# EMI-Group/evogp

Measured on AMD Instinct MI355X. Metric: tree_evals_per_s, higher is better.
Workload: dtype f32; 1 GPU; BASELINE north_star / configs[2] shape: SymbolicRegression synthetic 10-var, GLOBAL pop=1000000 x 1024 datapoints, max_tree_len=64, funcs + - * /, one tree_SR_fitness pass over every rank's shard per step; global_pop=1000000, pop_per_gpu=1000000, datapoints=1024, var_len=10, max_tree_len=64, ranks=1, device_prewarm_calls=40

## Files before the change

evogp_amd/_lib.py:

```python
from __future__ import annotations

import ctypes as C
import os

_HERE = os.path.dirname(os.path.abspath(__file__))
LIB_PATH = os.environ.get("EVOGP_HIP_LIB") or os.path.join(_HERE, "lib", "libevogp_hip.so")

ABI_VERSION = 9

_vp = C.c_void_p
_u = C.c_uint
_i = C.c_int
_f = C.c_float

PROTOTYPES = {
    "evogp_hip_generate": [_u, _u, _u, _u, _u, _f, _f, _vp, _vp, _vp, _vp, _vp, _vp, _vp, _u, _vp],
    "evogp_hip_mutate": [_i, _i, _vp, _vp, _vp, _vp, _vp, _vp, _vp, _vp, _vp, _vp, _vp],
    "evogp_hip_crossover": [_i, _i, _i, _vp, _vp, _vp, _vp, _vp, _vp, _vp, _vp, _vp, _vp, _vp],
    "evogp_hip_evaluate": [_u, _u, _u, _u, _vp, _vp, _vp, _vp, _vp, _vp],
    "evogp_hip_sr_fitness": [_u, _u, _u, _u, _u, _i, _vp, _vp, _vp, _vp, _vp, _vp, _u, _vp],
    "evogp_hip_generate_masked": [_u, _u, _u, _u, _u, _f, _f, _vp, _vp, _vp, _vp, _vp, _vp, _vp, _u, _vp, _u, _vp],
    "evogp_hip_breed_default": [_i, _i, _i, _i, _vp, _vp, _vp, _vp, _vp, _u, _vp, _vp, _vp, _vp, _vp, _vp, _vp, _vp],
    "evogp_hip_breed_default_rows": [_i, _i, _i, _i, _vp, _vp, _vp, _vp, _vp, _u, _vp, _vp, _vp, _vp, _vp, _vp, _vp, _i, _i, _vp],
    "evogp_hip_breed_default_table": [_i, _i, _i, _i, _i, _vp, _vp, _vp, _vp, _vp, _u, _vp, _vp, _vp, _vp, _vp, _vp, _vp, _i, _i, _vp],
# ... 34 lines not shown
    "evogp_hip_tree_hash": [_u, _u, _vp, _vp, _vp, _vp, _vp],
    "evogp_hip_tree_classes_workspace_bytes": [_u, C.POINTER(C.c_ulonglong)],
    "evogp_hip_tree_classes": [_u, _u, _vp, _vp, _vp, _vp, _vp, _vp, _vp],
    "evogp_hip_sr_semantic_hash_workspace_bytes": [_u, C.POINTER(C.c_ulonglong)],
    "evogp_hip_sr_semantic_hash": [_u, _u, _u, _u, _u, _vp, _vp, _vp, _vp, _vp, _vp, _vp],
    "evogp_hip_sr_semantic_classes_workspace_bytes": [_u, C.POINTER(C.c_ulonglong)],
    "evogp_hip_sr_semantic_classes": [_u, _u, _u, _u, _u, _vp, _vp, _vp, _vp, _vp, _vp, _vp, _vp],
    "evogp_hip_sr_linear_scaling": [_u, _u, _u, _u, _u, _vp, _vp, _vp, _vp, _vp, _vp, _vp, _vp],
    "evogp_hip_sr_weighted_loss": [_u, _u, _u, _u, _u, _vp, _vp, _vp, _vp, _vp, _vp, _u, _i, C.c_double, _vp, _vp],
    "evogp_hip_sr_weighted_gradient": [_u, _u, _u, _u, _u, _vp, _vp, _vp, _vp, _vp, _vp, _i, C.c_double, _vp, _vp, _vp],
    "evogp_hip_sr_weighted_normal_eq": [_u, _u, _u, _u, _u, _vp, _vp, _vp, _vp, _vp, _vp, _vp, _vp, _vp],
    "evogp_hip_sr_weighted_scaling": [_u, _u, _u, _u, _u, _vp, _vp, _vp, _vp, _vp, _vp, _u, _vp, _vp, _vp],
    "evogp_hip_sr_input_gradient": [_u, _u, _u, _u, _u, _vp, _vp, _vp, _vp, _u, _vp, _vp, _vp, _vp],
    "evogp_hip_sr_derivative_loss": [_u, _u, _u, _u, _u, _vp, _vp, _vp, _vp, _vp, _vp, _u, _vp, _vp, _vp, _vp, _vp, _vp],
    "evogp_hip_sr_gene_fitness": [_u, _u, _u, _u, _u, _vp, _vp, _vp, _vp, _vp, _vp, _vp, _vp, _vp],
    "evogp_hip_wrap_linear":[_u, _u, _u, _vp, _vp, _vp, _vp, _vp, _vp, _vp, _vp, _vp],
    "evogp_hip_tree_intervals": [_u, _u, _u, _vp, _vp, _vp, _vp, _vp, _vp, _vp, _vp, _vp],
    "evogp_hip_tree_derivative_intervals": [_u, _u, _u, _vp, _vp, _vp, _vp, _vp, _u, _vp, _vp, _vp, _vp, _vp, _vp, _vp, _vp],
    "evogp_hip_tree_dimensions": [_u, _u, _u, _u, _vp, _vp, _vp, _vp, _vp, _i, _vp, _vp, _vp, _vp],
    "evogp_hip_tree_structure": [_u, _u, _u, _vp, _vp, _vp, _vp, _vp, _vp, _vp, _vp, _i, _i, _vp, _vp, _vp, _vp, _vp, _vp, _vp],
}

DEBUG_PROTOTYPES = {
    "evogp_hip_timer_begin": [_vp],
    "evogp_hip_timer_end": [_vp, C.POINTER(C.c_float)],
    "evogp_hip_debug_set_stats": [_vp],
    "evogp_hip_debug_compile_batch": [_i],
    "evogp_hip_debug_long_compiler": [_i],
    "evogp_hip_debug_twins": [_i],
    "evogp_hip_debug_tc_fold": [_i],
    "evogp_hip_debug_tc_end": [_i],
    "evogp_hip_debug_tc_nanpeek": [_i],
    "evogp_hip_debug_tc_nanpeek_raised": [],
    "evogp_hip_debug_tc_batches": [_i, _i],
    "evogp_hip_debug_tc_table": [_i],
    "evogp_hip_debug_tc_dense": [_i],
    "evogp_hip_debug_tc_dense_fallbacks": [],
    "evogp_hip_debug_tc_table_entry": [_i, _i, C.POINTER(C.c_uint)],
    "evogp_hip_debug_profile": [_i],
    "evogp_hip_debug_profile_read": [C.POINTER(C.c_float), C.POINTER(C.c_int)],
    "evogp_hip_debug_tc_histogram": [_u, _vp, _i, _vp],
    "evogp_hip_debug_tc_nhandlers": [],
    "evogp_hip_debug_tc_program": [_u, _vp, _i],
    "evogp_hip_debug_forget_function_classes": [],
    "evogp_hip_debug_structural_mutate_given": [_i, _i, _i, _i, _i, _vp, _vp, _vp, _vp, _vp, _vp, _vp, _vp],
    "evogp_hip_debug_insert_mutate_given": [_i, _i, _i, _vp, _vp, _vp, _vp, _vp, _vp, _vp, _vp, _vp, _vp, _vp],
    "evogp_hip_debug_point_mutate_given": [_i, _i, _i, _i, _i, _i, _i, _i, _i, _vp, _vp, _vp, _vp, _vp, _vp, _vp, _vp, _vp, _vp, _vp, _vp, _vp, _vp],
    "evogp_hip_debug_lexicase": [_vp, _i],
    "evogp_hip_debug_pareto_rank": [_i],
}


def _load() -> C.CDLL:
    if not os.path.exists(LIB_PATH):
        raise ImportError(
            f"{LIB_PATH} is missing: build the HIP engine first "
            "(python -c 'import __graft_entry__ as g; g.build()'  or  make -C evogp_amd/csrc). "
            "evogp_amd has no CPU fallback."
        )
    lib = C.CDLL(LIB_PATH)
    for name, argtypes in list(PROTOTYPES.items()) + list(DEBUG_PROTOTYPES.items()):
        fn = getattr(lib, name)
        fn.argtypes = argtypes
        fn.restype = _i
    lib.evogp_hip_evaluate_workspace_bytes.argtypes = [_u, _u]
    lib.evogp_hip_evaluate_workspace_bytes.restype = C.c_size_t
# ... 21 lines not shown
```

evogp_amd/csrc/gen/gen_tc_asm.py:

```python
#!/usr/bin/env python3
import os
import sys

sys.path.insert(0, os.path.dirname(os.path.abspath(__file__)))
from ocml_bodies import BODIES
from pair_rows import Pairing, check as check_pairing

FORMS = ("SS", "SV", "VS", "SC", "CS", "VV", "VC", "CV")
SENTINEL_HEAVY = 0x7FC0FEED
OPS = ("add", "sub", "mul", "div")
UNARY = ("neg", "abs", "sin", "cos", "tan", "sqrt", "lsqrt", "exp", "log", "llog")
GBIN = ("ldiv", "max", "min", "lt", "gt", "le", "ge", "pow", "lpow")
GUN = ("zero", "sinh", "cosh", "tanh", "one", "rcp")
HEAVY_REGS = 24
SLOT = 256
DIVIP_REGS = 12
DIVIP = ("SS", "SC", "CS")
DIVR = ("SV", "VV", "CV")
NOPF_TWINS = tuple(f"{op}_{form}" for op in ("add", "sub", "mul") for form in FORMS) + ("push_c", "push_v") \
    + tuple(f"divip_{f}" for f in DIVIP) + tuple(f"divr_{f}" for f in DIVR)
NHF = 37 + 2 * len(UNARY) + 8 + 2 + 4 + len(DIVIP) + 1 + 1 + len(DIVR) + len(NOPF_TWINS) + 1 + 3


NOPF = False
SPLAT = False
FMA_LOSS = False
PKARITH = True
DIVABREAST = True
PKCONST = True
TRUST = True
DIVFIX = False
DIVRANGE = True
DIV_LO, DIV_HI = 0x28800000, 0x56800000
EARLYREC = True
L2WARM = True
KWARM_LINES = 4
FUSED_SIZE_OFF, FUSED_LEN_OFF = 96 + 16, 96 + 60
TOUCH = True
TRIGPK = True
LIBPK = True
RECGLC = False
CODEWARM = False
CNDE64 = False
NANPEEK_BIT = 15
KWARM = False


def count_path(L, start, taken, idx_on=True, stop=()):
    idx = {line[:-1]: i for i, line in enumerate(L) if line.endswith(":")}
    c = {"valu": 0, "trans": 0, "salu": 0, "lds": 0, "vmem": 0, "smem": 0, "valu_clk": 0}
    i, steps = idx[start], 0
    while steps < 20000:
        steps += 1
        line = L[i]
        i += 1
        if line.endswith(":") and line[:-1] in stop:
            break
        if line.endswith(":") or line.startswith("."):
            continue
        w = line.split()
        op = w[0]
        if op.startswith("v_"):
            c["valu"] += 1
            if op.split("_")[1] in ("rcp", "sqrt", "exp", "log", "rsq", "sin", "cos"):
                c["trans"] += 1
                c["valu_clk"] += 8
            else:
                srcs = " ".join(w[2:]) if len(w) > 2 else ""
                fast = not idx_on and op in ("v_add_f32", "v_sub_f32", "v_subrev_f32", "v_mul_f32", "v_mov_b32") and not any(
                    t in srcs for t in ("s", "0x", "|", "%"))
                c["valu_clk"] += 2 if fast else 4
        elif op.startswith("ds_"):
            c["lds"] += 1
        elif op.startswith("global_") or op.startswith("buffer_"):
            c["vmem"] += 1
        elif op.startswith("s_load") or op.startswith("s_memtime"):
            c["smem"] += 1
# ... 112 lines not shown
            a(f"s_lshr_b32 {PF}, s{sX}, 24")

    def read_aux(dst):
        a(f"s_movrels_b32 s{dst}, s{W}")
        a(f"s_bfe_u32 s{dst}, s{dst}, 0x80010")

    def prefetch(nxt):
        if NOPF or twin[0]:
            return
        a(f"v_lshl_add_u32 v4, {PF}, 10, v2")
        read_bank(nxt, 4)

    def warm(sreg):
        if not L2WARM:
            return
        a(f"s_mul_hi_u32 s{T2}, {sreg}, s19")
        a(f"s_mul_i32 s{T1}, {sreg}, s19")
        a(f"s_add_u32 s{T1}, s{T1}, s8")
        a(f"s_addc_u32 s{T2}, s{T2}, s9")
        a(f"global_load_dwordx4 v[14:17], v13, s[{T1}:{T2}]")
        a(f"global_load_dwordx4 v[14:17], v13, s[{T1}:{T2}] offset:1024")

    LIVE = "%[karg]"

    def batch_size(end):
        a(f"s_sub_u32 s{sNB}, {end}, s{sT0}")
        dyn_batch(T1)
        a(f"s_min_u32 s{sNB}, s{sNB}, s{T1}")
        if peek:
            a(f"s_bfm_b64 {LIVE}, s{sNB}, 0")
            a(f"s_cmp_lt_u32 s{sNB}, 64")
            a(f"s_cselect_b64 {LIVE}, {LIVE}, -1")

    def peek_issue():
        skip = lab(f"no_peek_{len(sect[0])}")
        a(f"s_bitcmp1_b32 s17, {NANPEEK_BIT}")
        a(f"s_cbranch_scc0 {skip}")
        rec_addr(T1, T2, f"s{sT0}", T1)
        a("v_mul_lo_u32 v5, v0, s19")
        a(f"s_mov_b64 exec, {LIVE}")
        a(f"global_load_dword v18, v5, s[{T1}:{T2}]")
        a("s_mov_b64 exec, -1")
        a(f"{skip}:")

    def next_live(none):
        a(f"s_cmp_eq_u64 {LIVE}, 0")
        a(f"s_cbranch_scc1 {none}")
        a(f"s_ff1_i32_b64 s{sB}, {LIVE}")
        a(f"s_bitset0_b64 {LIVE}, s{sB}")

    def next_in_batch(none):
        if peek:
            a(f"s_cmp_eq_u64 {LIVE}, 0")
            a(f"s_cbranch_scc1 {none}")
            a(f"s_ff1_i32_b64 s{T2}, {LIVE}")
        else:
            a(f"s_add_u32 s{T2}, s{sB}, 1")
            a(f"s_cmp_lt_u32 s{T2}, s{sNB}")
            a(f"s_cbranch_scc0 {none}")

    def dyn_batch(dst):
        a(f"s_bfe_u32 s{T2}, s17, 0x20008")
        a(f"s_lshr_b32 s{dst}, s16, s{T2}")
        a(f"s_max_u32 s{dst}, s{dst}, 1")

    def grab():
        dyn_batch(T1)
        a("s_mov_b64 exec, 1")
        a(f"v_mov_b32 v9, s{T1}")
        a("global_atomic_add v12, v[10:11], v9, off sc0")
        a("s_mov_b64 exec, -1")

    def pool_grab():
        dyn_batch(T1)
# ... 66 lines not shown
        a(f"s_load_dwordx2 s[{P3_}:{P4_}], %[karg], 0x10")
        a("s_load_dwordx8 s[12:19], %[karg], 0x28")
        a("s_waitcnt lgkmcnt(0)")
        a(f"s_or_b32 s17, s17, {BASE}")
        a(f"v_mov_b32 v10, s{P3_}")
        a(f"v_mov_b32 v11, s{P4_}")
        a("s_mul_i32 s14, s14, s15")
        a(f"s_mul_i32 s14, s14, {G * 1024}")
        a("v_lshrrev_b32 v13, 4, v0")
        a("v_mul_lo_u32 v13, v13, s19")
        a("v_and_b32 v9, 15, v0")
        a("v_lshl_add_u32 v13, v9, 4, v13")
        a(f"s_load_dwordx4 s[{P1_}:{P4_}], %[karg], 0x48")
        a("s_waitcnt lgkmcnt(0)")
        a(f"s_mul_i32 {CUR}, {CUR}, s{P1_}")
        a(f"s_add_u32 {END_}, {CUR}, s{P1_}")
        a(f"s_mov_b32 {DYN}, s{P2_}")
        a(f"s_getreg_b32 s{P1_}, hwreg(HW_REG_XCC_ID, 0, 4)")
        a(f"s_bfe_u32 s{P2_}, s17, 0x3000c")
        a(f"s_and_b32 s{P1_}, s{P1_}, s{P2_}")
        a(f"s_mul_i32 s{P2_}, s{P1_}, s18")
        a(f"s_add_u32 {DYN}, {DYN}, s{P2_}")
        a(f"s_add_u32 s{P2_}, {DYN}, s18")
        a(f"s_min_u32 s12, s12, s{P2_}")
        a(f"s_lshl_b32 s{P1_}, s{P1_}, 7")
        a(f"v_add_co_u32 v10, vcc, s{P1_}, v10")
        a("v_addc_co_u32 v11, vcc, 0, v11, vcc")
        a(f"s_getpc_b64 s[{T1}:{T2}]")
        a(f"{lab('pc')}:")
        a(f"s_add_u32 s{T1}, s{T1}, {lab('hbase')}-{lab('pc')}")
        a(f"s_addc_u32 s{T2}, s{T2}, 0")
        a(f"s_mov_b32 {BASE}, s{T1}")
        a(f"s_mov_b32 s{sPC + 1}, s{T2}")
        if CODEWARM:
            a("v_lshlrev_b32 v4, 6, v0")
            a(f"s_mov_b32 s{P3_}, ({lab('code_end')}-{lab('hbase')}+4095)/4096")
            a(f"{lab('codewarm')}:")
            a(f"global_load_dword v14, v4, s[{T1}:{T2}]")
            a(f"s_add_u32 s{T1}, s{T1}, 4096")
            a(f"s_addc_u32 s{T2}, s{T2}, 0")
            a(f"s_sub_u32 s{P3_}, s{P3_}, 1")
            a(f"s_cmp_lg_u32 s{P3_}, 0")
            a(f"s_cbranch_scc1 {lab('codewarm')}")
        a(f"{lab('run')}:")
        if stats:
            for r in (A_REC, A_WORK, A_TREES, A_DISP):
                a(f"v_mov_b32 v{r}, 0")
            a(f"s_memtime s[{T1}:{T2}]")
            a("s_waitcnt lgkmcnt(0)")
            a(f"v_mov_b32 v{A_START}, s{T1}")
        a("s_mov_b32 s18, 1")
        pool_grab()
        a("s_waitcnt lgkmcnt(0)")
        a(f"v_readfirstlane_b32 s{sT0N}, v12")
        a(f"s_add_u32 s{sT0N}, s{sT0N}, {CUR}")
        a(f"{lab('batch')}:")
        a("s_cmp_eq_u32 s18, 0")
        a(f"s_cbranch_scc1 {lab('dyn')}")
        a(f"s_mov_b32 s{sT0}, s{sT0N}")
        a(f"s_cmp_lt_u32 s{sT0}, {END_}")
        a(f"s_cbranch_scc0 {lab('to_dyn')}")
        if peek:
            batch_size(END_)
            peek_issue()
        pool_grab()
        warm(f"s{sT0}")
# ... 4 lines not shown
        a("s_mov_b32 s18, 0")
        tick_begin()
        grab()
        a("s_waitcnt vmcnt(0)")
        tick_end(A_WORK)
        a(f"v_readfirstlane_b32 s{sT0N}, v12")
        a(f"s_add_u32 s{sT0N}, s{sT0N}, {DYN}")
        a(f"{lab('dyn')}:")
        a(f"s_mov_b32 s{sT0}, s{sT0N}")
        a(f"s_cmp_ge_u32 s{sT0}, s12")
        a(f"s_cbranch_scc1 {lab('exit')}")
        if peek:
            batch_size("s12")
            peek_issue()
        grab()
        warm(f"s{sT0}")
        if not peek:
            batch_size("s12")
    a(f"{lab('have_batch')}:")
    a(f"s_mov_b64 s[{sOK}:{sOK + 1}], 0")
    a("v_mov_b32 v7, 0")
    if peek:
        nw = 2 if L2WARM else 0
        a(f"s_mov_b32 s{sNB}, 0")
        a(f"s_bitcmp1_b32 s17, {NANPEEK_BIT}")
        a(f"s_cbranch_scc0 {lab('first_tree')}")
        a("s_cmp_eq_u32 s18, 1")
        a(f"s_cbranch_scc1 {lab('peek_pool')}")
        a(f"s_waitcnt vmcnt({nw + 1})")
        a(f"s_branch {lab('peek_here')}")
        a(f"{lab('peek_pool')}:")
        a(f"s_waitcnt vmcnt({nw})")
        a(f"{lab('peek_here')}:")
        a("v_and_b32 v18, 0xffff, v18")
        a(f"v_cmp_eq_u32 vcc, {hex(SLOT * hid['nan_tree'])}, v18")
        a("v_mov_b32 v9, 0x7fc00000")
        a(f"s_and_b64 vcc, vcc, {LIVE}")
        a(f"s_andn2_b64 {LIVE}, {LIVE}, vcc")
        a(f"s_mov_b64 s[{sOK}:{sOK + 1}], vcc")
        a("s_nop 1")
        a("v_cndmask_b32 v7, v7, v9, vcc")
        a(f"{lab('first_tree')}:")
        next_live(lab('batch_end'))
    else:
        a(f"s_mov_b32 s{sB}, 0")
    a(f"{lab('tree')}:")
    if fused:
        rec_addr(sREC, sREC + 1, f"s{sB}", T1)
    else:
        a(f"s_add_u32 s{T1}, s{sT0}, s{sB}")
        rec_addr(sREC, sREC + 1, f"s{T1}", T1)
    tick_begin()
    load_window()
    a(f"{lab('tree_loaded')}:")
    a("v_mov_b32 v6, 0")
    a(f"s_mov_b32 s{sTILE}, 0")
    a("s_waitcnt lgkmcnt(0)")
    tick_end(A_REC)
    if not fused:
        if peek:
            a(f"s_add_u32 s{sNB}, s{sNB}, 1")
            a(f"s_cmp_eq_u32 s{sNB}, 2")
        else:
            a(f"s_cmp_eq_u32 s{sB}, 1")
        a(f"s_cbranch_scc0 {lab('no_prewarm')}")
        a("s_cmp_eq_u32 s18, 1")
        a(f"s_cbranch_scc0 {lab('no_prewarm')}")
        second_tree_hook("", lab('no_prewarm'))
        a(f"{lab('no_prewarm')}:")
    if stats:
        a(f"v_add_u32 v{A_TREES}, 1, v{A_TREES}")
    elif KWARM and not fused:
        for i in range(KWARM_LINES):
            a(f"s_load_dwordx2 %[karg], s[{sREC}:{sREC + 1}], {hex(256 + 64 * i)}")
# ... 1625 lines not shown
        if x is not None:
            rows_op("sub", y, y, x)
        elif PKCONST and K >= 2:
            for k in range(0, K, 2):
                a(f"v_pk_add_f32 v[{y + k}:{y + k + 1}], v[{y + k}:{y + k + 1}], s[{sA}:{sA + 1}] op_sel_hi:[1,0] neg_lo:[0,1] neg_hi:[0,1]")
        else:
            for k in range(K):
                a(f"v_subrev_f32 v{y + k}, s{sA}, v{y + k}")
        rows_op("mul", y, y, y)
        for k in range(K):
            a(f"v_add_f32 v6, v6, v{y + k}")

    for fl in (0, 1):
        a(f"{lab(f'lean_last{fl}')}:")
        early_record(f"lean{fl}")
        rows_op("sub", S0, P[fl], S0)
        rows_op("mul", S0, S0, S0)
        for k in range(K):
            a(f"v_add_f32 v6, v6, v{S0 + k}")
        a(f"s_branch {lab('tree_done')}")
        a(f"{lab(f'lean_moved{fl}')}:")
        a("s_bitset0_b32 s17, 31")
        if fused:
            rec_addr(sREC, sREC + 1, f"s{sB}", T1)
        else:
            a(f"s_add_u32 s{T1}, s{sT0}, s{sB}")
            rec_addr(sREC, sREC + 1, f"s{T1}", T1)
        load_window()
        rows_op("mul", S0, S0, S0)
        for k in range(K):
            a(f"v_add_f32 v6, v6, v{S0 + k}")
        a("s_waitcnt lgkmcnt(0)")
        a(f"s_branch {lab('tile')}")
    for leaf in ("leaf_c", "leaf_v"):
        var = leaf == "leaf_v"
        Xb, Yb = ((P[0], P[1]) if var else (None, None)), (T, Q)
        for ph in (0, 1):
            a(f"{lab(f'{leaf}_p{ph}')}:")
            a(f"s_add_u32 s{sTILE}, s{sTILE}, 1")
            a(f"s_cmp_lt_u32 s{sTILE}, s15")
            a(f"s_cbranch_scc0 {lab(f'{leaf}_last{ph}')}")
            if var:
                a(f"v_add_u32 v4, {G * 1024}, v4")
                read_bank(Xb[1 - ph], 4)
            a(f"v_add_u32 v3, {G * 1024}, v3")
            read_bank(Yb[1 - ph], 3)
            a(f"s_waitcnt lgkmcnt({(2 if var else 1) * G})")
            mse_rows(Yb[ph], Xb[ph])
            if ph == 1:
                a(f"s_branch {lab(f'{leaf}_p0')}")
        for ph in (0, 1):
            a(f"{lab(f'{leaf}_last{ph}')}:")
            a("s_waitcnt lgkmcnt(0)")
            early_record(f"{leaf}{ph}")
            mse_rows(Yb[ph], Xb[ph])
            a(f"s_branch {lab('tree_done')}")

    for fl in (0, 1):
        Y = P[fl]
        a(f"{lab(f'endbody{fl}')}:")
        a("s_set_gpr_idx_off")
        if stats:
            pass
        a(f"s_add_u32 s{T1}, s{sTILE}, 1")
        a("s_waitcnt lgkmcnt(0)")
        if EARLYREC and not stats:
            a(f"s_cmp_lt_u32 s{T1}, s15")
            a(f"s_cbranch_scc1 {lab(f'no_early{fl}')}")
            next_in_batch(lab(f'no_early{fl}'))
            if not fused:
                a(f"s_add_u32 s{T2}, s{T2}, s{sT0}")
            rec_addr(sREC, sREC + 1, f"s{T2}", T2)
            load_window()
            a(f"{lab(f'no_early{fl}')}:")
        a(f"s_and_b32 s{T2}, s17, 0x12")
        a(f"s_cbranch_scc0 {lab(f'end_full{fl}')}")
        a(f"s_cmp_lt_u32 s{T1}, s15")
        a(f"s_cselect_b32 s{T2}, 0, s17")
        a("s_bitcmp1_b32 s17, 4")
        a(f"s_cselect_b32 s{T2}, s17, s{T2}")
        a(f"s_and_b32 s{T2}, s{T2}, 2")
        a("s_waitcnt lgkmcnt(0)")
        a(f"s_cmp_eq_u32 s{T2}, 0")
        a(f"s_cbranch_scc1 {lab(f'end_full{fl}')}")
        a(f"s_mul_i32 s{T2}, s{sTILE}, {64 * K}")
        a(f"v_mul_u32_u24 v5, {RPL}, v0")
        for k in range(K):
            g, q = divmod(k, 4)
            a(f"s_add_u32 s{T4}, s{T2}, {g * 256 + q}")
# ... 18 lines not shown
        else:
            for k in range(K):
                a(f"v_sub_f32 v{S0 + k}, v{Y + k}, v{S0 + k}")
            for k in range(K):
                a(f"v_mul_f32 v{S0 + k}, v{S0 + k}, v{S0 + k}")
            for k in range(K):
                a(f"v_add_f32 v6, v6, v{S0 + k}")
        a(f"s_branch {lab('end_acc')}")
        a(f"{lab(f'end_abs{fl}')}:")
        for k in range(K):
            a(f"v_sub_f32 v{S0 + k}, v{Y + k}, v{S0 + k}")
        for k in range(K):
            a(f"v_add_f32_e64 v6, v6, |v{S0 + k}|")
        if fl == 0:
            a(f"s_branch {lab('end_acc')}")
    a(f"{lab('end_acc')}:")
    a(f"s_mov_b32 s{sTILE}, s{T1}")
    a(f"s_cmp_lt_u32 s{sTILE}, s15")
    a(f"s_cbranch_scc0 {lab('tree_done')}")
    if fused:
        rec_addr(T1, T2, f"s{sB}", T1)
    else:
        a(f"s_add_u32 s{T1}, s{sT0}, s{sB}")
        rec_addr(T1, T2, f"s{T1}", T1)
    a(f"s_cmp_eq_u32 s{T1}, s{sREC}")
    a(f"s_cbranch_scc1 {lab('tile')}")
    a(f"s_mov_b32 s{sREC}, s{T1}")
    a(f"s_mov_b32 s{sREC + 1}, s{T2}")
    load_window()
    a("s_waitcnt lgkmcnt(0)")
    a(f"s_branch {lab('tile')}")
    a(f"{lab('tree_done')}:")
    a("s_bitset0_b32 s17, 31")
    for ctl in ("row_shr:1 row_mask:0xf bank_mask:0xf bound_ctrl:0", "row_shr:2 row_mask:0xf bank_mask:0xf bound_ctrl:0",
                "row_shr:4 row_mask:0xf bank_mask:0xf bound_ctrl:0", "row_shr:8 row_mask:0xf bank_mask:0xf bound_ctrl:0",
                "row_bcast:15 row_mask:0xa bank_mask:0xf", "row_bcast:31 row_mask:0xc bank_mask:0xf"):
        a("s_nop 1")
        a(f"v_add_f32_dpp v6, v6, v6 {ctl}")
    a("s_nop 1")
    a(f"v_readlane_b32 s{T1}, v6, 63")
    a(f"s_and_b32 s{T2}, s{T1}, 0x7fffffff")
    a(f"s_cmp_gt_u32 s{T2}, 0x7f800000")
    a(f"s_cselect_b32 s{T1}, 0x7fc00000, s{T1}")
    a(f"s_mov_b32 m0, s{sB}")
    a(f"s_bitset1_b64 s[{sOK}:{sOK + 1}], s{sB}")
    a(f"v_writelane_b32 v7, s{T1}, m0")
    if EARLYREC and not stats:
        if peek:
            next_live(lab('batch_end'))
        else:
            a(f"s_add_u32 s{sB}, s{sB}, 1")
            a(f"s_cmp_lt_u32 s{sB}, s{sNB}")
            a(f"s_cbranch_scc0 {lab('batch_end')}")
        a("s_bitcmp1_b32 s17, 10")
        a(f"s_cbranch_scc1 {lab('tree_loaded')}")
        a(f"s_branch {lab('tree')}")
    a(f"{lab('next_tree')}:")
    if peek:
        next_live(lab('batch_end'))
        a(f"s_branch {lab('tree')}")
    else:
        a(f"s_add_u32 s{sB}, s{sB}, 1")
        a(f"s_cmp_lt_u32 s{sB}, s{sNB}")
        a(f"s_cbranch_scc1 {lab('tree')}")
    a(f"{lab('batch_end')}:")
    if peek:
        a(f"s_bitcmp1_b32 s17, {NANPEEK_BIT}")
        a(f"s_cbranch_scc0 {lab('hooked')}")
        a(f"s_cmp_ge_u32 s{sNB}, 2")
        a(f"s_cbranch_scc1 {lab('hooked')}")
        a("s_cmp_eq_u32 s18, 1")
        a(f"s_cbranch_scc0 {lab('hooked')}")
        a("s_waitcnt lgkmcnt(0)")
        second_tree_hook("_end", lab('hooked'))
        a(f"{lab('hooked')}:")
    tick_begin()
    if fused:
        a("s_waitcnt vmcnt(0)")
    else:
# ... 176 lines not shown
```

evogp_amd/csrc/sr_tc.hip:

```cpp
#include "interp.hpp"
#include "launch.hpp"
#include "sr_params.hpp"
#include "tc_interp_k8.inc"
#include "tc_interp_k4.inc"
#include "tc_interp_k1.inc"

#include <atomic>
#include <cstddef>
#include <mutex>
#include <cstdio>
#include <vector>

namespace evogp {

struct TcCompileParams {
    const float *value;
    const int16_t *type;
    const int16_t *size;
    uint2 *prog;
    float *fitness;
    unsigned *marks;
    unsigned *zero_next;
    int pop, gp_len, var_len;
    uint32_t unary_mask;
// ... 6 lines not shown
    int nblocks;
    int rows;
    int general;
    int heavy_reserve;
    int div_reserve;
    int classify;
    uint32_t recip;
    int twins;
    int long_fast;
    int learn;
    int nan_trees;
    int end_id;
    int leaf_id;
};

__device__ inline uint32_t division_in_place(uint32_t id, int after, const TcCompileParams &p) {
    if (id < 24u || id >= 32u) return id;
    const uint32_t form = id - 24u;
    const uint32_t ip = form == 0u ? (uint32_t)EVOGP_TC_H_DIVIP_SS : form == 3u ? (uint32_t)EVOGP_TC_H_DIVIP_SC : form == 4u ? (uint32_t)EVOGP_TC_H_DIVIP_CS : 0u;
    if (ip == 0u) return id;
    const int before = after + (form == 0u ? 1 : 0);
    return before + p.div_reserve <= p.depth ? ip : id;
}

enum : int { TC_S = 0, TC_V = 1, TC_C = 2 };
constexpr int kMarkSampleBlocks = 64;
constexpr int kZeroRounds = 3;
static std::atomic<int> g_long_fast{-1};
static std::atomic<int> g_twins{-1};
static std::atomic<int> g_fold{-1};
static std::atomic<int> g_lean_end{-1};
static std::atomic<int> g_nanpeek{-1};
static std::atomic<int> g_nanpeek_raised{0};
static std::atomic<int> g_tc_batch{0}, g_tc_dynshift{-1};
static std::atomic<int> g_compile_batch{-2};
static std::atomic<int> g_word_table{-1};
static int tc_nan_trees() {
    static const int env_fold = env_int("EVOGP_TC_FOLD", 2);
    const int fo = g_fold.load(std::memory_order_relaxed);
    return fo >= 0 ? fo : (env_fold < 0 || env_fold > 2 ? 2 : env_fold);
}
static bool tc_lean_end() {
    static const int env_end = env_int("EVOGP_TC_END", 1);
    const int le = g_lean_end.load(std::memory_order_relaxed);
    return (le >= 0 ? le : env_end) != 0;
}
static bool tc_nanpeek(long n, int num_cus) {
    static const int env_peek = env_int("EVOGP_TC_NANPEEK", 1);
    const int np = g_nanpeek.load(std::memory_order_relaxed);
    return np >= 0 ? np != 0 : (env_peek == 2 || (env_peek == 1 && n >= 900l * num_cus));
}
static bool tc_word_table() {
    static const int env_table = env_int("EVOGP_TC_TABLE", 1);
    const int wt = g_word_table.load(std::memory_order_relaxed);
    return (wt >= 0 ? wt : env_table) != 0;
}
static std::atomic<int> g_dense{-1};
static bool tc_dense() {
    static const int env_dense = env_int("EVOGP_TC_DENSE", 1);
    const int de = g_dense.load(std::memory_order_relaxed);
    return (de >= 0 ? de : env_dense) != 0;
}
static std::atomic<unsigned *> g_dense_fallbacks{nullptr};
static_assert(EVOGP_TC_H_LEAF_V == EVOGP_TC_H_LEAF_C + 1, "TcCompileParams::leaf_id: the variable's word is the constant's + 1, as PUSH_V is PUSH_C + 1");
static_assert(kSentinelHeavy == 0x7FC0FEEDu, "gen/gen_tc_asm.py SENTINEL_HEAVY");

__device__ inline float fold_bin4_fast(int op, float x, float y) {
    return op == 0 ? x + y : op == 1 ? x - y : op == 2 ? x * y : (y == 0.0f ? __builtin_nanf("") : x / y);
}

__device__ inline uint32_t tc_word0(int id, int slot, uint32_t pf_bytes, uint32_t aux = 0u) {
    return ((pf_bytes >> 10) << 24) | ((aux & 0xFFu) << 16) | (uint32_t)(((slot & 1) * EVOGP_TC_NHANDLERS + id) * EVOGP_TC_SLOT);
}

static_assert(EVOGP_TC_H_PUSH_V == EVOGP_TC_H_PUSH_C + 1 && EVOGP_TC_H_DIVIP_CS == EVOGP_TC_H_DIVIP_SS + 2 && EVOGP_TC_H_DIVR_CV == EVOGP_TC_H_DIVR_SV + 2 &&
              EVOGP_TC_H_PUSH_C_NP == EVOGP_TC_H_ADD_SS_NP + 24 && EVOGP_TC_H_DIVIP_SS_NP == EVOGP_TC_H_ADD_SS_NP + 26 &&
              EVOGP_TC_H_DIVR_SV_NP == EVOGP_TC_H_ADD_SS_NP + 29, "gen/gen_tc_asm.py NOPF_TWINS");
__device__ inline int no_prefetch_delta(bool arith3, bool push_c, bool in_place, bool by_recip) {
    return arith3 ? (int)EVOGP_TC_H_ADD_SS_NP : push_c ? (int)EVOGP_TC_H_PUSH_C_NP - (int)EVOGP_TC_H_PUSH_C
         : in_place ? (int)EVOGP_TC_H_DIVIP_SS_NP - (int)EVOGP_TC_H_DIVIP_SS : by_recip ? (int)EVOGP_TC_H_DIVR_SV_NP - (int)EVOGP_TC_H_DIVR_SV : 0;
}
__device__ inline bool next_word_has_variable(const TcCompileParams &, unsigned long long keptwave, bool kept, bool uses_var, bool is_root) {
    const unsigned long long U = __ballot(kept & uses_var);
// ... 3247 lines not shown
        if (marks) {
            marks += (size_t)piece * kCallScratchChunkWords;
            t.counter = marks + 32;
            t.flags |= 1 << 16;
            regions = xcc_regions(stream);
            if (regions > kCallScratchXcds) regions = kCallScratchXcds;
            if ((env_xcc == 1 || env_xcc == 2 || env_xcc == 4 || env_xcc == 8) && env_xcc <= regions) regions = env_xcc;
        } else {
            t.counter = acquire_counter(strm, &le);
            if (!t.counter) return le;
        }
        long blocks = (long)info.num_cus * wgs_per_cu;
        const long grain = std::max(1, batch >> dyn_shift);
        const long need_blocks = ((long)n + grain * wg_waves - 1) / (grain * wg_waves);
        if (blocks > need_blocks) blocks = need_blocks;
        int static_pct = K == 1 ? 50 : n < 200000 ? 85 : 75;
        if (env_static >= 0 && env_static <= 100) static_pct = env_static;
        t.static_per_wg = (uint32_t)(((long)n * static_pct / 100) / blocks);
        t.dyn_start = t.static_per_wg * (uint32_t)blocks;
        t.waves_per_wg = (uint32_t)wg_waves;
        {
            const long tail = (long)n - (long)t.dyn_start;
            while (regions > 1 && (long)regions > blocks) regions >>= 1;
            if (tail < (long)regions * batch * 4) regions = 1;
            long per = (tail + regions - 1) / regions;
            per = (per + batch - 1) / batch * batch;
            t.reserved = (int)per;
            static_assert(kCallScratchXcds <= 8, "TcParams::flags bits 12-14");
            t.flags |= (regions - 1) << 12;
        }
        const bool may_divide = p.func_mask == 0u || (p.func_mask & (1u << F_DIV)) != 0u;
        if (!STATS && !WIDE && nan_words && may_divide && tc_nanpeek(n, info.num_cus)) t.flags |= 1 << 15;
        g_nanpeek_raised.store((t.flags >> 15) & 1, std::memory_order_relaxed);
        unsigned *publish = marks && piece == 0 && pieces == 1 && chunks == 1 && learn_packed ? p.feedback : nullptr;
        hipLaunchKernelGGL((sr_tc_kernel<K, STATS, FAST, WIDE>), dim3((unsigned)blocks), dim3(wg_waves * 64), lds, strm, t, publish, p.feedback_expected,
                           div_magic((unsigned)t.var_len), div_magic((t.pad & 0xFFFFu) > 0u ? (t.pad & 0xFFFFu) : 1u));
        return hipGetLastError();
    };

    if (p.classify) {
        int *cls = (int *)(records + cls_off);
        hipLaunchKernelGGL(tc_label_groups_kernel, dim3(1), dim3(1024), 0, stream, (const int *)p.y, p.D, p.out_len, K, piece_rows, (int)cls_q,
                           cls, cls + p.D, cls + p.D + cls_q);
        const int nxp = (int)cls_q * p.var_len;
        hipLaunchKernelGGL(tc_permute_rows_kernel, dim3((unsigned)((nxp + 1023) / 1024)), dim3(256), 0, stream, p.X, (const int *)(cls + p.D),
                           (float *)(cls + p.D + 2 * cls_q), p.var_len, nxp);
        if ((e = hipGetLastError()) != hipSuccess) return e;
    }
    if (chunks == 1) {
        if ((e = launch_compilers(0, p.pop, p.marks, true, stream)) != hipSuccess) return e;
        if (p.zero_next) call_scratch_next_is_clean(stream);
        if (p.prof_mid) (void)hipEventRecord(p.prof_mid, stream);
        for (int piece = 0; piece < pieces; ++piece)
            if ((e = launch_interpreter(0, p.pop, p.marks, stream, piece)) != hipSuccess) return e;
        if (pieces > 1 && !p.classify) {
            hipLaunchKernelGGL(tc_scale_kernel, dim3((unsigned)((p.pop + 255) / 256)), dim3(256), 0, stream, p.fitness, p.pop, (float)p.D);
            if ((e = hipGetLastError()) != hipSuccess) return e;
        }
    } else {
        if ((e = hipEventRecord(d.fork, stream)) != hipSuccess) return e;
        if ((e = hipStreamWaitEvent(d.side, d.fork, 0)) != hipSuccess) return e;
        for (int c = 0; c < chunks; ++c) {
            const int lo = (int)((long)p.pop * c / chunks), hi = (int)((long)p.pop * (c + 1) / chunks);
            unsigned *cm = p.marks + (size_t)c * kCallScratchChunkWords;
            if ((e = launch_compilers(lo, hi - lo, cm, c == 0, d.side)) != hipSuccess) return e;
            if ((e = hipEventRecord(d.ready[c], d.side)) != hipSuccess) return e;
// ... 330 lines not shown
extern "C" int evogp_hip_debug_twins(int mode) {
    if (mode < -1 || mode > 1) return EVOGP_E_BADARG;
    evogp::g_twins.store(mode, std::memory_order_relaxed);
    return EVOGP_OK;
}

extern "C" int evogp_hip_debug_tc_fold(int mode) {
    if (mode < -1 || mode > 2) return EVOGP_E_BADARG;
    evogp::g_fold.store(mode, std::memory_order_relaxed);
    return EVOGP_OK;
}

extern "C" int evogp_hip_debug_tc_end(int mode) {
    if (mode < -1 || mode > 1) return EVOGP_E_BADARG;
    evogp::g_lean_end.store(mode, std::memory_order_relaxed);
    return EVOGP_OK;
}

extern "C" int evogp_hip_debug_tc_nanpeek(int mode) {
    if (mode < -1 || mode > 1) return EVOGP_E_BADARG;
    evogp::g_nanpeek.store(mode, std::memory_order_relaxed);
    return EVOGP_OK;
}

extern "C" int evogp_hip_debug_tc_batches(int batch, int dyn_shift) {
    if (batch < 0 || batch > 64 || dyn_shift < -1 || dyn_shift > 3) return EVOGP_E_BADARG;
    evogp::g_tc_batch.store(batch, std::memory_order_relaxed);
    evogp::g_tc_dynshift.store(dyn_shift, std::memory_order_relaxed);
    return EVOGP_OK;
}

extern "C" int evogp_hip_debug_tc_nanpeek_raised(void) { return evogp::g_nanpeek_raised.load(std::memory_order_relaxed); }

extern "C" int evogp_hip_debug_tc_table(int mode) {
    if (mode < -1 || mode > 1) return EVOGP_E_BADARG;
    evogp::g_word_table.store(mode, std::memory_order_relaxed);
    return EVOGP_OK;
}

extern "C" int evogp_hip_debug_tc_dense(int mode) {
    if (mode < -1 || mode > 1) return EVOGP_E_BADARG;
    evogp::g_dense.store(mode, std::memory_order_relaxed);
    return EVOGP_OK;
}

extern "C" int evogp_hip_debug_tc_dense_fallbacks(void) {
    const unsigned *const word = evogp::g_dense_fallbacks.load(std::memory_order_relaxed);
    unsigned n = 0u;
    if (!word || hipDeviceSynchronize() != hipSuccess || hipMemcpy(&n, word, sizeof n, hipMemcpyDeviceToHost) != hipSuccess) return -1;
    return (int)n;
}

extern "C" int evogp_hip_debug_tc_table_entry(int recip, int code, unsigned *entry) {
    if (recip < 0 || recip > 1 || code < 0 || code >= evogp::kTcCodes || !entry) return EVOGP_E_BADARG;
    entry[0] = evogp::kTcWordTableHost.ids[recip][code];
    entry[1] = evogp::kTcWordTableHost.bits[recip][code];
    return EVOGP_OK;
}

extern "C" int evogp_hip_debug_long_compiler(int fast) {
    if (fast < -1 || fast > 1) return EVOGP_E_BADARG;
    evogp::g_long_fast.store(fast, std::memory_order_relaxed);
    return EVOGP_OK;
}

extern "C" int evogp_hip_debug_compile_batch(int trees) {
// ... 104 lines not shown
```

include/evogp_hip_debug.h:

```cpp
#ifndef EVOGP_HIP_DEBUG_H
#define EVOGP_HIP_DEBUG_H
#include "evogp_hip.h"
#ifdef __cplusplus
extern "C" {
#endif

int evogp_hip_timer_begin(evogp_stream_t stream);
int evogp_hip_timer_end(evogp_stream_t stream, float *elapsed_ms);

int evogp_hip_debug_set_stats(unsigned long long *device_counters);

int evogp_hip_debug_profile(int enable);
int evogp_hip_debug_profile_read(float *stage_ms , int *calls);

int evogp_hip_debug_compile_batch(int trees);
int evogp_hip_debug_long_compiler(int fast);
int evogp_hip_debug_twins(int mode);
int evogp_hip_debug_tc_fold(int mode);
int evogp_hip_debug_tc_end(int mode);
int evogp_hip_debug_tc_nanpeek(int mode);
int evogp_hip_debug_tc_nanpeek_raised(void);
int evogp_hip_debug_tc_batches(int batch, int dyn_shift);
int evogp_hip_debug_tc_table(int mode);
int evogp_hip_debug_tc_dense(int mode);
int evogp_hip_debug_tc_dense_fallbacks(void);
int evogp_hip_debug_tc_table_entry(int recip, int code, unsigned *entry);

int evogp_hip_debug_tc_histogram(unsigned pop, unsigned long long *device_hist, int hist_len, evogp_stream_t stream);
int evogp_hip_debug_tc_nhandlers(void);
int evogp_hip_debug_tc_program(unsigned tree, unsigned *host_words, int max_words);

int evogp_hip_debug_forget_function_classes(void);

int evogp_hip_debug_structural_mutate_given(int pop_size, int gp_len, int mode, int inner_is_offset, int skip_rows, const int *given,
                                            const float *value, const int16_t *type, const int16_t *size, float *value_res,
                                            int16_t *type_res, int16_t *size_res, evogp_stream_t stream);
int evogp_hip_debug_insert_mutate_given(int pop_size, int gp_len, int skip_rows, const int *given, const float *value, const int16_t *type,
                                        const int16_t *size, const float *donor_value, const int16_t *donor_type, const int16_t *donor_size,
                                        float *value_res, int16_t *type_res, int16_t *size_res, evogp_stream_t stream);
int evogp_hip_debug_point_mutate_given(int pop_size, int gp_len, int mode, int modify_output, int fix_roulette, int skip_rows, int input_len,
                                       int output_len, int n_consts, const unsigned char *target, const float *u, const int *var_idx,
                                       const int *const_idx, const int *out_idx, const float *value, const int16_t *type, const int16_t *size,
                                       const float *roulette_ufuncs, const float *roulette_bfuncs, const float *roulette_tfuncs,
                                       const float *const_samples, float *value_res, evogp_stream_t stream);

int evogp_hip_debug_lexicase(unsigned long long *device_counters, int stop_after);

int evogp_hip_debug_pareto_rank(int stop_after);

#ifdef __cplusplus
}
#endif
#endif
```

Baseline: 1990 billion tree-evals/s.

## Peek tree roots to batch-evaluate single-leaf trees in a dedicated walk loop

Extends the NaN-peek preload in the generated SR fitness assembly so it also spots trees whose root is a lone constant or variable leaf. It loads an extra word per tree and flags these trees, then evaluates them in a separate leaf-walk loop that reuses the leaf MSE tile bodies and skips the normal interpreter dispatch. The path is gated on population size and lean-end mode, and it can be toggled by an environment variable or a debug call. It adds code size and branch complexity, and it packs a flag into the low bit of the code base register.

```diff
diff --git a/evogp_amd/_lib.py b/evogp_amd/_lib.py
--- a/evogp_amd/_lib.py
+++ b/evogp_amd/_lib.py
@@ -90,6 +90,8 @@
     "evogp_hip_debug_tc_end": [_i],
     "evogp_hip_debug_tc_nanpeek": [_i],
     "evogp_hip_debug_tc_nanpeek_raised": [],
+    "evogp_hip_debug_tc_leafpeek": [_i],
+    "evogp_hip_debug_tc_leafpeek_raised": [],
     "evogp_hip_debug_tc_batches": [_i, _i],
     "evogp_hip_debug_tc_table": [_i],
     "evogp_hip_debug_tc_dense": [_i],
diff --git a/evogp_amd/csrc/gen/gen_tc_asm.py b/evogp_amd/csrc/gen/gen_tc_asm.py
--- a/evogp_amd/csrc/gen/gen_tc_asm.py
+++ b/evogp_amd/csrc/gen/gen_tc_asm.py
@@ -43,6 +43,7 @@
 CODEWARM = False
 CNDE64 = False
 NANPEEK_BIT = 15
+LEAFPEEK_PAD_BIT = 17
 KWARM = False
 
 
@@ -221,14 +222,23 @@
             a(f"s_cmp_lt_u32 s{sNB}, 64")
             a(f"s_cselect_b64 {LIVE}, {LIVE}, -1")
 
+    def leafpeek_test():
+        a(f"s_bitcmp1_b32 {BASE}, 0")
+
     def peek_issue():
-        skip = lab(f"no_peek_{len(sect[0])}")
+        skip, wide = lab(f"no_peek_{len(sect[0])}"), lab(f"peek_x2_{len(sect[0])}")
         a(f"s_bitcmp1_b32 s17, {NANPEEK_BIT}")
         a(f"s_cbranch_scc0 {skip}")
         rec_addr(T1, T2, f"s{sT0}", T1)
         a("v_mul_lo_u32 v5, v0, s19")
         a(f"s_mov_b64 exec, {LIVE}")
+        leafpeek_test()
+        a(f"s_cbranch_scc1 {wide}")
         a(f"global_load_dword v18, v5, s[{T1}:{T2}]")
+        a("s_mov_b64 exec, -1")
+        a(f"s_branch {skip}")
+        a(f"{wide}:")
+        a(f"global_load_dwordx2 v[18:19], v5, s[{T1}:{T2}]")
         a("s_mov_b64 exec, -1")
         a(f"{skip}:")
 
@@ -361,6 +371,9 @@
         a(f"s_addc_u32 s{T2}, s{T2}, 0")
         a(f"s_mov_b32 {BASE}, s{T1}")
         a(f"s_mov_b32 s{sPC + 1}, s{T2}")
+        if peek:
+            a(f"s_bfe_u32 s{P4_}, s{P4_}, {hex(0x10000 | LEAFPEEK_PAD_BIT)}")
+            a(f"s_or_b32 {BASE}, {BASE}, s{P4_}")
         if CODEWARM:
             a("v_lshlrev_b32 v4, 6, v0")
             a(f"s_mov_b32 s{P3_}, ({lab('code_end')}-{lab('hbase')}+4095)/4096")
@@ -431,14 +444,24 @@
         a(f"{lab('peek_pool')}:")
         a(f"s_waitcnt vmcnt({nw})")
         a(f"{lab('peek_here')}:")
-        a("v_and_b32 v18, 0xffff, v18")
-        a(f"v_cmp_eq_u32 vcc, {hex(SLOT * hid['nan_tree'])}, v18")
+        a("v_and_b32 v5, 0xffff, v18")
+        a(f"v_cmp_eq_u32 vcc, {hex(SLOT * hid['nan_tree'])}, v5")
         a("v_mov_b32 v9, 0x7fc00000")
         a(f"s_and_b64 vcc, vcc, {LIVE}")
         a(f"s_andn2_b64 {LIVE}, {LIVE}, vcc")
         a(f"s_mov_b64 s[{sOK}:{sOK + 1}], vcc")
         a("s_nop 1")
         a("v_cndmask_b32 v7, v7, v9, vcc")
+        leafpeek_test()
+        a(f"s_cbranch_scc0 {lab('first_tree')}")
+        a(f"v_cmp_eq_u32 vcc, {hex(SLOT * hid['leaf_c'])}, v5")
+        a(f"s_mov_b32 s{sA}, {hex(SLOT * hid['leaf_v'])}")
+        a(f"v_cmp_eq_u32 s[{T1}:{T2}], s{sA}, v5")
+        a(f"s_or_b64 vcc, vcc, s[{T1}:{T2}]")
+        a(f"s_and_b64 s[{sJ}:{sJ + 1}], vcc, {LIVE}")
+        a(f"s_andn2_b64 {LIVE}, {LIVE}, s[{sJ}:{sJ + 1}]")
+        a(f"s_cmp_lg_u64 s[{sJ}:{sJ + 1}], 0")
+        a(f"s_cbranch_scc1 {lab('leaf_walk')}")
         a(f"{lab('first_tree')}:")
         next_live(lab('batch_end'))
     else:
@@ -2130,14 +2153,14 @@
             a(f"v_add_f32 v6, v6, v{S0 + k}")
         a("s_waitcnt lgkmcnt(0)")
         a(f"s_branch {lab('tile')}")
-    for leaf in ("leaf_c", "leaf_v"):
+    def leaf_body(leaf, tag, last_tile, done):
         var = leaf == "leaf_v"
         Xb, Yb = ((P[0], P[1]) if var else (None, None)), (T, Q)
         for ph in (0, 1):
-            a(f"{lab(f'{leaf}_p{ph}')}:")
+            a(f"{lab(f'{tag}{leaf}_p{ph}')}:")
             a(f"s_add_u32 s{sTILE}, s{sTILE}, 1")
             a(f"s_cmp_lt_u32 s{sTILE}, s15")
-            a(f"s_cbranch_scc0 {lab(f'{leaf}_last{ph}')}")
+            a(f"s_cbranch_scc0 {lab(f'{tag}{leaf}_last{ph}')}")
             if var:
                 a(f"v_add_u32 v4, {G * 1024}, v4")
                 read_bank(Xb[1 - ph], 4)
@@ -2146,13 +2169,74 @@
             a(f"s_waitcnt lgkmcnt({(2 if var else 1) * G})")
             mse_rows(Yb[ph], Xb[ph])
             if ph == 1:
-                a(f"s_branch {lab(f'{leaf}_p0')}")
+                a(f"s_branch {lab(f'{tag}{leaf}_p0')}")
         for ph in (0, 1):
-            a(f"{lab(f'{leaf}_last{ph}')}:")
+            a(f"{lab(f'{tag}{leaf}_last{ph}')}:")
             a("s_waitcnt lgkmcnt(0)")
-            early_record(f"{leaf}{ph}")
+            last_tile(ph)
             mse_rows(Yb[ph], Xb[ph])
-            a(f"s_branch {lab('tree_done')}")
+            a(f"s_branch {done}")
+
+    for leaf in ("leaf_c", "leaf_v"):
+        leaf_body(leaf, "", lambda ph, leaf=leaf: early_record(f"{leaf}{ph}"), lab('tree_done'))
+
+    def tree_result():
+        for ctl in ("row_shr:1 row_mask:0xf bank_mask:0xf bound_ctrl:0", "row_shr:2 row_mask:0xf bank_mask:0xf bound_ctrl:0",
+                    "row_shr:4 row_mask:0xf bank_mask:0xf bound_ctrl:0", "row_shr:8 row_mask:0xf bank_mask:0xf bound_ctrl:0",
+                    "row_bcast:15 row_mask:0xa bank_mask:0xf", "row_bcast:31 row_mask:0xc bank_mask:0xf"):
+            a("s_nop 1")
+            a(f"v_add_f32_dpp v6, v6, v6 {ctl}")
+        a("s_nop 1")
+        a(f"v_readlane_b32 s{T1}, v6, 63")
+        a(f"s_and_b32 s{T2}, s{T1}, 0x7fffffff")
+        a(f"s_cmp_gt_u32 s{T2}, 0x7f800000")
+        a(f"s_cselect_b32 s{T1}, 0x7fc00000, s{T1}")
+        a(f"s_mov_b32 m0, s{sB}")
+        a(f"s_bitset1_b64 s[{sOK}:{sOK + 1}], s{sB}")
+        a(f"v_writelane_b32 v7, s{T1}, m0")
+
+    if peek:
+        F = f"s[{sJ}:{sJ + 1}]"
+        a(f"{lab('leaf_walk')}:")
+        a(f"s_ff1_i32_b64 s{sB}, {F}")
+        a(f"s_bitset0_b64 {F}, s{sB}")
+        a(f"v_readlane_b32 s{T1}, v18, s{sB}")
+        a(f"v_readlane_b32 s{sA}, v19, s{sB}")
+        a("v_mov_b32 v6, 0")
+        a(f"s_mov_b32 s{sTILE}, 0")
+        a("v_add_u32 v3, s14, v1")
+        a(f"s_and_b32 s{T2}, s{T1}, 0xffff")
+        a(f"s_cmp_eq_u32 s{T2}, {hex(SLOT * hid['leaf_v'])}")
+        a(f"s_cbranch_scc1 {lab('leaf_walk_v')}")
+        read_bank(T, 3)
+        a(f"s_branch {lab('w_leaf_c_p0')}")
+        a(f"{lab('leaf_walk_v')}:")
+        a(f"s_lshr_b32 {PF}, s{T1}, 24")
+        a(f"v_lshl_add_u32 v4, {PF}, 10, v1")
+        read_bank(P[0], 4)
+        read_bank(T, 3)
+        a(f"s_branch {lab('w_leaf_v_p0')}")
+
+        def walk_last_tile(leaf, ph):
+            if not EARLYREC:
+                return
+            a(f"s_cmp_lg_u64 {F}, 0")
+            a(f"s_cbranch_scc1 {lab(f'no_early_w_{leaf}{ph}')}")
+            early_record(f"w_{leaf}{ph}")
+
+        for leaf in ("leaf_c", "leaf_v"):
+            leaf_body(leaf, "w_", lambda ph, leaf=leaf: walk_last_tile(leaf, ph), lab('leaf_walk_done'))
+        a(f"{lab('leaf_walk_done')}:")
+        tree_result()
+        a(f"s_cmp_lg_u64 {F}, 0")
+        a(f"s_cbranch_scc1 {lab('leaf_walk')}")
+        if EARLYREC:
+            next_live(lab('batch_end'))
+            a("s_bitcmp1_b32 s17, 10")
+            a(f"s_cbranch_scc1 {lab('tree_loaded')}")
+            a(f"s_branch {lab('tree')}")
+        else:
+            a(f"s_branch {lab('next_tree')}")
 
     for fl in (0, 1):
         Y = P[fl]
@@ -2237,19 +2321,7 @@
     a(f"s_branch {lab('tile')}")
     a(f"{lab('tree_done')}:")
     a("s_bitset0_b32 s17, 31")
-    for ctl in ("row_shr:1 row_mask:0xf bank_mask:0xf bound_ctrl:0", "row_shr:2 row_mask:0xf bank_mask:0xf bound_ctrl:0",
-                "row_shr:4 row_mask:0xf bank_mask:0xf bound_ctrl:0", "row_shr:8 row_mask:0xf bank_mask:0xf bound_ctrl:0",
-                "row_bcast:15 row_mask:0xa bank_mask:0xf", "row_bcast:31 row_mask:0xc bank_mask:0xf"):
-        a("s_nop 1")
-        a(f"v_add_f32_dpp v6, v6, v6 {ctl}")
-    a("s_nop 1")
-    a(f"v_readlane_b32 s{T1}, v6, 63")
-    a(f"s_and_b32 s{T2}, s{T1}, 0x7fffffff")
-    a(f"s_cmp_gt_u32 s{T2}, 0x7f800000")
-    a(f"s_cselect_b32 s{T1}, 0x7fc00000, s{T1}")
-    a(f"s_mov_b32 m0, s{sB}")
-    a(f"s_bitset1_b64 s[{sOK}:{sOK + 1}], s{sB}")
-    a(f"v_writelane_b32 v7, s{T1}, m0")
+    tree_result()
     if EARLYREC and not stats:
         if peek:
             next_live(lab('batch_end'))
diff --git a/evogp_amd/csrc/sr_tc.hip b/evogp_amd/csrc/sr_tc.hip
--- a/evogp_amd/csrc/sr_tc.hip
+++ b/evogp_amd/csrc/sr_tc.hip
@@ -62,6 +62,8 @@
 static std::atomic<int> g_lean_end{-1};
 static std::atomic<int> g_nanpeek{-1};
 static std::atomic<int> g_nanpeek_raised{0};
+static std::atomic<int> g_leafpeek{-1};
+static std::atomic<int> g_leafpeek_raised{0};
 static std::atomic<int> g_tc_batch{0}, g_tc_dynshift{-1};
 static std::atomic<int> g_compile_batch{-2};
 static std::atomic<int> g_word_table{-1};
@@ -79,6 +81,11 @@
     static const int env_peek = env_int("EVOGP_TC_NANPEEK", 1);
     const int np = g_nanpeek.load(std::memory_order_relaxed);
     return np >= 0 ? np != 0 : (env_peek == 2 || (env_peek == 1 && n >= 900l * num_cus));
+}
+static bool tc_leafpeek(long n, int num_cus) {
+    static const int env_leaf = env_int("EVOGP_TC_LEAFPEEK", 1);
+    const int lp = g_leafpeek.load(std::memory_order_relaxed);
+    return lp >= 0 ? lp != 0 : (env_leaf == 2 || (env_leaf == 1 && n >= 1900l * num_cus));
 }
 static bool tc_word_table() {
     static const int env_table = env_int("EVOGP_TC_TABLE", 1);
@@ -3392,6 +3399,9 @@
         const bool may_divide = p.func_mask == 0u || (p.func_mask & (1u << F_DIV)) != 0u;
         if (!STATS && !WIDE && nan_words && may_divide && tc_nanpeek(n, info.num_cus)) t.flags |= 1 << 15;
         g_nanpeek_raised.store((t.flags >> 15) & 1, std::memory_order_relaxed);
+        const bool leafpeek = lean_end && tc_leafpeek(n, info.num_cus);
+        if (leafpeek) { t.pad |= 1u << 17; t.flags |= 1 << 15; }
+        g_leafpeek_raised.store(leafpeek ? 1 : 0, std::memory_order_relaxed);
         unsigned *publish = marks && piece == 0 && pieces == 1 && chunks == 1 && learn_packed ? p.feedback : nullptr;
         hipLaunchKernelGGL((sr_tc_kernel<K, STATS, FAST, WIDE>), dim3((unsigned)blocks), dim3(wg_waves * 64), lds, strm, t, publish, p.feedback_expected,
                            div_magic((unsigned)t.var_len), div_magic((t.pad & 0xFFFFu) > 0u ? (t.pad & 0xFFFFu) : 1u));
@@ -3788,6 +3798,14 @@
 
 extern "C" int evogp_hip_debug_tc_nanpeek_raised(void) { return evogp::g_nanpeek_raised.load(std::memory_order_relaxed); }
 
+extern "C" int evogp_hip_debug_tc_leafpeek(int mode) {
+    if (mode < -1 || mode > 1) return EVOGP_E_BADARG;
+    evogp::g_leafpeek.store(mode, std::memory_order_relaxed);
+    return EVOGP_OK;
+}
+
+extern "C" int evogp_hip_debug_tc_leafpeek_raised(void) { return evogp::g_leafpeek_raised.load(std::memory_order_relaxed); }
+
 extern "C" int evogp_hip_debug_tc_table(int mode) {
     if (mode < -1 || mode > 1) return EVOGP_E_BADARG;
     evogp::g_word_table.store(mode, std::memory_order_relaxed);
diff --git a/include/evogp_hip_debug.h b/include/evogp_hip_debug.h
--- a/include/evogp_hip_debug.h
+++ b/include/evogp_hip_debug.h
@@ -20,6 +20,8 @@
 int evogp_hip_debug_tc_end(int mode);
 int evogp_hip_debug_tc_nanpeek(int mode);
 int evogp_hip_debug_tc_nanpeek_raised(void);
+int evogp_hip_debug_tc_leafpeek(int mode);
+int evogp_hip_debug_tc_leafpeek_raised(void);
 int evogp_hip_debug_tc_batches(int batch, int dyn_shift);
 int evogp_hip_debug_tc_table(int mode);
 int evogp_hip_debug_tc_dense(int mode);
```

Result: no change. 2001 billion tree-evals/s (median of 6 runs) (+0.5%).
